# uibk-uncover/ws-unet

Hardware: AMD Instinct MI355X
Metric: 512x512 grayscale images/sec (UNet predict) (higher is better)
Workload: dtype f16 MFMA on the f16 halves + ONE block-scaled fp4 (e2m1) MFMA per tap pair for both residual cross terms (per-pixel / per-(co, tap) E8M0 scales), fp32 accumulate; planar storage

## Files before the change

ws_unet_amd/csrc/planar.hip:

```cpp
#include "wsu_device.h"

namespace {

typedef __attribute__((address_space(3))) void lds_void;
typedef __attribute__((address_space(1))) const void glb_void;

__device__ __forceinline__ void swap32(uint32_t& upper_of, uint32_t& lower_of) {
    const auto r = __builtin_amdgcn_permlane32_swap(upper_of, lower_of, false, false);
    upper_of = r[0]; lower_of = r[1];
}

__device__ __forceinline__ void store_chunk_px(const f32x4& X, const f32x4& Y, char* dst, size_t plane_bytes, int hh, bool ok, float div_lo = WSU_F8_XLO_DIV, bool with_res = true) {
    uint32_t xh0, xh1, xlo, yh0, yh1, ylo;
    wsu_split4_f16r8(X, div_lo, xh0, xh1, xlo);
    wsu_split4_f16r8(Y, div_lo, yh0, yh1, ylo);
    swap32(xh0, yh0); swap32(xh1, yh1);
    uint32_t xlp = xlo, ylp = ylo;
    swap32(xlo, xlp); swap32(ylo, ylp);
    if (ok) {
        *reinterpret_cast<u32x4*>(dst + hh * plane_bytes) = mk_u4(xh0, xh1, yh0, yh1);
        if (with_res && !hh) *reinterpret_cast<u32x4*>(dst + 2 * plane_bytes) = mk_u4(xlo, xlp, ylo, ylp);
    }
}

// ... 386 lines not shown
            const int yy = min(irow, a.h - 1), xx = min(icol, a.w - 1);
#pragma unroll
            for (int cp = 0; cp < 2; ++cp)
#pragma unroll
                for (int pl = 0; pl < 2; ++pl)
                    mk[cp][pl] = *reinterpret_cast<const u32x2*>(a.mask + ((((size_t)cur.n * nci + cur.cb * 4 + mh * 2 + cp) * 3 + pl) * hw + (size_t)yy * a.w + xx) * 16 + hh * 8);
        }
        const char* ldsA = st + GEO::IN1 + (mh * 32 + l31) * 16;
        const char* ldsB = st + (row * 64 + 2 * l31) * 16;
        auto boff = [](int plane, int sub) constexpr { return (((plane * 2 + (sub >> 1)) * 4) * 64 + (sub & 1)) * 16; };
        if constexpr (HONLY) {
#pragma unroll
            for (int s2 = 0; s2 < 4; ++s2) {
                const u32x4 ah = *reinterpret_cast<const u32x4*>(ldsA + ((s2 * 2 + hh) * 64) * 16);
                const u32x4 bh = *reinterpret_cast<const u32x4*>(ldsB + boff(hh, s2));
                wsu_mfma_f16(ah, bh, acc);
            }
        } else {
#pragma unroll
        for (int t = 0; t < 2; ++t) {
            const int s = 2 * t + hh;
            const u32x4 a0 = *reinterpret_cast<const u32x4*>(ldsA + ((s * 4 + 2) * 64) * 16), a1 = *reinterpret_cast<const u32x4*>(ldsA + ((s * 4 + 3) * 64) * 16);
            const u32x4 b0 = *reinterpret_cast<const u32x4*>(ldsB + boff(2, s)), b1 = *reinterpret_cast<const u32x4*>(ldsB + boff(3, s));
            wsu_mfma_f8x2(a0, a1, b0, b1, sc_a, sc_b, acc);
#pragma unroll
            for (int u = 0; u < 2; ++u) {
                const int s2 = 2 * t + u;
                const u32x4 ah = *reinterpret_cast<const u32x4*>(ldsA + ((s2 * 4 + hh) * 64) * 16);
                const u32x4 bh = *reinterpret_cast<const u32x4*>(ldsB + boff(hh, s2));
                wsu_mfma_f16(ah, bh, acc);
            }
        }
        }
        if (c + 1 == a.nch) {
            const bool ok = irow < a.h && icol < a.w;
#pragma unroll
            for (int cp = 0; cp < 2; ++cp) {
                const int oc = cur.cb * 4 + mh * 2 + cp;
                f32x4 X, Y;
#pragma unroll
                for (int e = 0; e < 4; ++e) { X[e] = acc[8 * cp + e]; Y[e] = acc[8 * cp + 4 + e]; }
                if (a.mask) {
#pragma unroll
                    for (int e = 0; e < 4; ++e) {
                        const uint32_t wx = e < 2 ? mk[cp][0].x : mk[cp][0].y, wy = e < 2 ? mk[cp][1].x : mk[cp][1].y;
                        const short hx = (short)((e & 1) ? wx >> 16 : wx & 0xFFFF), hy = (short)((e & 1) ? wy >> 16 : wy & 0xFFFF);
                        if (!(hx > 0)) X[e] = 0.f;
                        if (!(hy > 0)) Y[e] = 0.f;
                    }
                }
                char* dst = a.dx + ((((size_t)cur.n * nci + oc) * 3) * hw + (size_t)min(irow, a.h - 1) * a.w + min(icol, a.w - 1)) * 16;
                store_chunk_px(X, Y, dst, hw * 16, hh, ok, WSU_F8_GLO_DIV, !HONLY);
            }
            ++kt; c = 0;
            if (j + 1 < J) cur = ctb_tile_of(a, lw + kt * G);
        } else {
            ++c;
        }
    }
}

__global__ void pack_convt_dgrad_pl_kernel(const float* __restrict__ w, char* __restrict__ dst, int cin, int cout) {
    const int nch = cout / 16;
    const long long total = (long long)(cin / WSU_COB) * nch * 4 * WSU_COB;
    for (long long d = (long long)blockIdx.x * blockDim.x + threadIdx.x; d < total; d += (long long)gridDim.x * blockDim.x) {
        long long t = d;
        const int m = t % WSU_COB; t /= WSU_COB;
        const int sub = t % 4; t /= 4;
        const int c = t % nch; const int cb = (int)(t / nch);
        f32x4 q[4];
#pragma unroll
        for (int e = 0; e < 16; ++e) q[e >> 2][e & 3] = w[(((size_t)(cb * WSU_COB + m) * cout + c * 16 + e) * 2 + (sub >> 1)) * 2 + (sub & 1)];
        uint32_t h[8], l[4], x[4];
#pragma unroll
        for (int k = 0; k < 4; ++k) wsu_split4_f16f8(q[k], WSU_F8_WLO_DIV, WSU_F8_W_DIV, h[2 * k], h[2 * k + 1], l[k], x[k]);
        char* base = dst + (((size_t)cb * nch + c) * 4 + sub) * (4 * WSU_COB * 16) + m * 16;
        *reinterpret_cast<u32x4*>(base) = mk_u4(h[0], h[1], h[2], h[3]);
        *reinterpret_cast<u32x4*>(base + WSU_COB * 16) = mk_u4(h[4], h[5], h[6], h[7]);
        *reinterpret_cast<u32x4*>(base + 2 * WSU_COB * 16) = mk_u4(x[0], x[1], x[2], x[3]);
        *reinterpret_cast<u32x4*>(base + 3 * WSU_COB * 16) = mk_u4(l[0], l[1], l[2], l[3]);
    }
}

struct FirstPlArgs { const float* x; const float* w; const float* b; char* y; unsigned* range_flag; int n, h, w_, cin, cout, relu; unsigned char* relu_mask_out; int yq; };

template <int FMT, int CINMAX>
__global__ __launch_bounds__(256) void first_pl_kernel(const FirstPlArgs a) {
    constexpr bool YQ = FMT == WSU_PLANAR_Q;
    extern __shared__ __attribute__((aligned(16))) char smem[];
    float* wl = reinterpret_cast<float*>(smem);
    float* bl = wl + a.cin * 9 * a.cout;
    for (int i = threadIdx.x; i < a.cin * 9 * a.cout; i += blockDim.x) {
        const int co = i % a.cout, tap = (i / a.cout) % 9, ci = i / (9 * a.cout);
        wl[i] = a.w[((size_t)co * a.cin + ci) * 9 + tap];
    }
    for (int i = threadIdx.x; i < a.cout; i += blockDim.x) bl[i] = a.b ? a.b[i] : 0.f;
    __syncthreads();
    const size_t hw = (size_t)a.h * a.w_;
    const long long total = (long long)a.n * hw;
    const int nco = a.cout >> 4;
    float vmax = 0.f;
    for (long long i = (long long)blockIdx.x * blockDim.x + threadIdx.x; i < total; i += (long long)gridDim.x * blockDim.x) {
        const int x = (int)(i % a.w_); long long t = i / a.w_;
        const int y = (int)(t % a.h); const int img = (int)(t / a.h);
        float p[CINMAX][9];
#pragma unroll
        for (int ci = 0; ci < CINMAX; ++ci)
            if (ci < a.cin) {
                const float* src = a.x + ((size_t)img * a.cin + ci) * hw;
#pragma unroll
                for (int tp = 0; tp < 9; ++tp)
                    p[ci][tp] = src[(size_t)wsu_reflect(y + tp / 3 - 1, a.h) * a.w_ + wsu_reflect(x + tp % 3 - 1, a.w_)];
            }
        for (int oc = 0; oc < nco; ++oc) {
            f32x2 acc2[8];
#pragma unroll
            for (int k = 0; k < 8; ++k) acc2[k] = *reinterpret_cast<const f32x2*>(bl + oc * 16 + 2 * k);
#pragma unroll
            for (int ci = 0; ci < CINMAX; ++ci)
                if (ci < a.cin)
#pragma unroll
                    for (int tp = 0; tp < 9; ++tp) {
                        const float* wr = wl + (ci * 9 + tp) * a.cout + oc * 16;
                        const f32x2 pw = {p[ci][tp & ~1], p[ci][(tp | 1) < 9 ? (tp | 1) : tp]};
#pragma unroll
                        for (int g = 0; g < 4; ++g) {
                            const f32x4 w4 = *reinterpret_cast<const f32x4*>(wr + 4 * g);
                            const f32x2 wlo = {w4[0], w4[1]}, whi = {w4[2], w4[3]};
                            if (tp & 1) {
                                asm volatile("v_pk_fma_f32 %0, %1, %2, %0 op_sel:[1,0,0] op_sel_hi:[1,1,1]" : "+v"(acc2[2 * g]) : "v"(pw), "v"(wlo));
                                asm volatile("v_pk_fma_f32 %0, %1, %2, %0 op_sel:[1,0,0] op_sel_hi:[1,1,1]" : "+v"(acc2[2 * g + 1]) : "v"(pw), "v"(whi));
                            } else {
                                asm volatile("v_pk_fma_f32 %0, %1, %2, %0 op_sel:[0,0,0] op_sel_hi:[0,1,1]" : "+v"(acc2[2 * g]) : "v"(pw), "v"(wlo));
                                asm volatile("v_pk_fma_f32 %0, %1, %2, %0 op_sel:[0,0,0] op_sel_hi:[0,1,1]" : "+v"(acc2[2 * g + 1]) : "v"(pw), "v"(whi));
                            }
                        }
                    }
            asm volatile("s_nop 0" ::: "memory");
            f32x4 v[4];
#pragma unroll
            for (int g = 0; g < 4; ++g) v[g] = mk_f4(acc2[2 * g][0], acc2[2 * g][1], acc2[2 * g + 1][0], acc2[2 * g + 1][1]);
            uint32_t h[8], lo[4];
#pragma unroll
            for (int g = 0; g < 4; ++g) {
                if (a.relu) {
#pragma unroll
                    for (int e = 0; e < 4; ++e) v[g][e] = fmaxf(v[g][e], 0.f);
                }
#pragma unroll
                for (int e = 0; e < 4; ++e) vmax = fmaxf(vmax, fabsf(v[g][e]));
            }
            if constexpr (YQ) {
                u32x4 h0, h1, qg; uint32_t sb;
                wsu_q4_encode16(v, h0, h1, qg, sb);
                char* chunk = a.y + ((size_t)img * nco + oc) * wsu_q_chunk_bytes(a.h, a.w_);
                char* dq = chunk + ((size_t)y * a.w_ + x) * 16;
                *reinterpret_cast<u32x4*>(dq) = h0;
                *reinterpret_cast<u32x4*>(dq + hw * 16) = h1;
                *reinterpret_cast<u32x4*>(dq + 2 * hw * 16) = qg;
                *reinterpret_cast<unsigned char*>(chunk + 3 * hw * 16 + wsu_q_soff(y, x, (a.w_ + 31) >> 5)) = (unsigned char)sb;
                continue;
            }
            if constexpr (FMT == WSU_PLANAR_H) {
#pragma unroll
                for (int g = 0; g < 4; ++g) {
                    const f32x2 p0 = {v[g][0], v[g][1]}, p1 = {v[g][2], v[g][3]};
                    h[2 * g] = __builtin_bit_cast(uint32_t, __builtin_convertvector(p0, f16x2)); h[2 * g + 1] = __builtin_bit_cast(uint32_t, __builtin_convertvector(p1, f16x2));
                }
                char* dh = a.y + ((size_t)img * nco + oc) * wsu_h_chunk_bytes(a.h, a.w_) + ((size_t)y * a.w_ + x) * 16;
                *reinterpret_cast<u32x4*>(dh) = mk_u4(h[0], h[1], h[2], h[3]);
                *reinterpret_cast<u32x4*>(dh + hw * 16) = mk_u4(h[4], h[5], h[6], h[7]);
                continue;
            }
#pragma unroll
            for (int g = 0; g < 4; ++g) wsu_split4_f16r8(v[g], WSU_F8_XLO_DIV, h[2 * g], h[2 * g + 1], lo[g]);
            char* dst = a.y + ((((size_t)img * nco + oc) * 3) * hw + (size_t)y * a.w_ + x) * 16;
            *reinterpret_cast<u32x4*>(dst) = mk_u4(h[0], h[1], h[2], h[3]);
            *reinterpret_cast<u32x4*>(dst + hw * 16) = mk_u4(h[4], h[5], h[6], h[7]);
            *reinterpret_cast<u32x4*>(dst + 2 * hw * 16) = mk_u4(lo[0], lo[1], lo[2], lo[3]);
            if (a.relu_mask_out) {
                unsigned char* m = a.relu_mask_out + (((size_t)img * (nco * 2) + oc * 2) * wsu_mask_hp(a.h) + y) * wsu_mask_wp(a.w_) + x;
                m[0] = (unsigned char)wsu_f16x8_pos_bits(mk_u4(h[0], h[1], h[2], h[3]));
                m[(size_t)wsu_mask_hp(a.h) * wsu_mask_wp(a.w_)] = (unsigned char)wsu_f16x8_pos_bits(mk_u4(h[4], h[5], h[6], h[7]));
            }
        }
    }
    if (a.range_flag && !(vmax <= (FMT == WSU_PLANAR_H ? WSU_F16_RANGE : WSU_F8_RANGE))) atomicOr(a.range_flag, 1u);
}

}

extern "C" {

int wsu_convt2x2_pl_fwd(const void* x, const void* w_packed, const float* bias, void* y, int n, int h, int w, int cin, int cout,
                        int y_format, unsigned* range_flag, void* stream) {
    WSU_REQUIRE(y_format == WSU_PLANAR_A || y_format == WSU_PLANAR_Q, "convt2x2_pl: y_format must be WSU_PLANAR_A or WSU_PLANAR_Q");
    WSU_REQUIRE(x && w_packed && y, "convt2x2_pl: null pointer");
    WSU_REQUIRE(n > 0 && h > 0 && w > 0, "convt2x2_pl: bad shape n=%d h=%d w=%d", n, h, w);
    WSU_REQUIRE(cin > 0 && cin % 32 == 0, "convt2x2_pl: cin=%d must be a multiple of 32", cin);
    WSU_REQUIRE(cout > 0 && cout % WSU_COB == 0 && cout <= 1024, "convt2x2_pl: cout=%d must be a multiple of %d (<= 1024)", cout, WSU_COB);
    WSU_REQUIRE((long long)h * w * 200 < 0xFFFFFFF0LL, "convt2x2_pl: h*w too large (two input chunks and one output chunk must stay below 4 GiB)");
    CtpArgs a;
    a.x = (const char*)x; a.wp = (const char*)w_packed; a.bias = bias; a.y = (char*)y; a.range_flag = range_flag;
    a.n = n; a.h = h; a.w = w; a.cin = cin; a.cout = cout; a.yq = y_format == WSU_PLANAR_Q ? 1 : 0;
    a.tiles_x = (w + ct::TW - 1) / ct::TW; a.tiles_y = (h + ct::TH - 1) / ct::TH; a.ncb = cout / WSU_COB; a.nst = cin / 32;
    const long long nt = (long long)n * a.tiles_x * a.tiles_y * a.ncb;
    WSU_REQUIRE(nt > 0 && nt < 0x3FFFFFFFLL, "convt2x2_pl: %lld tiles out of range", nt);
    a.ntiles = (int)nt;
    const int ncu = wsu_cu_count("convt2x2_pl");
    if (!ncu) return WSU_ERR_HIP;
    static bool attr_done = false;
    if (!attr_done) {
        if (int rc = wsu_raise_lds(convt2x2_pl_kernel<false>, ct::LDS_TOTAL, "convt2x2_pl")) return rc;
        if (int rc = wsu_raise_lds(convt2x2_pl_kernel<true>, ct::LDS_TOTAL, "convt2x2_pl")) return rc;
        attr_done = true;
    }
    const int grid = (int)(nt < ncu ? nt : ncu);
    if (a.yq) hipLaunchKernelGGL(convt2x2_pl_kernel<true>, dim3(grid), dim3(ct::NT), ct::LDS_TOTAL, static_cast<hipStream_t>(stream), a);
    else hipLaunchKernelGGL(convt2x2_pl_kernel<false>, dim3(grid), dim3(ct::NT), ct::LDS_TOTAL, static_cast<hipStream_t>(stream), a);
    return wsu_check_launch("convt2x2_pl_kernel");
}

int wsu_convt2x2_pl_pack_dgrad(const float* w_iohw, void* w_packed, int cin, int cout, void* stream) {
    WSU_REQUIRE(w_iohw && w_packed, "convt2x2_pl_pack_dgrad: null pointer");
    WSU_REQUIRE(cin > 0 && cin % WSU_COB == 0 && cout > 0 && cout % 16 == 0, "convt2x2_pl_pack_dgrad: bad channels cin=%d cout=%d", cin, cout);
    hipLaunchKernelGGL(pack_convt_dgrad_pl_kernel, dim3(256), dim3(256), 0, static_cast<hipStream_t>(stream), w_iohw, (char*)w_packed, cin, cout);
    return wsu_check_launch("pack_convt_dgrad_pl_kernel");
}

int wsu_convt2x2_pl_bwd_data(const void* dy, const void* w_packed_dgrad, void* dx, const void* mask,
                             int n, int h, int w, int cin, int cout, int products, void* stream) {
    WSU_REQUIRE(dy && w_packed_dgrad && dx, "convt2x2_pl_bwd_data: null pointer");
    WSU_REQUIRE(products == WSU_PRODUCTS_F16F8 || products == WSU_PRODUCTS_F16, "convt2x2_pl_bwd_data: products must be WSU_PRODUCTS_F16F8 or WSU_PRODUCTS_F16");
    WSU_REQUIRE(n > 0 && h > 0 && w > 0 && cin > 0 && cin % WSU_COB == 0 && cout > 0 && cout % 16 == 0, "convt2x2_pl_bwd_data: bad shape (cin %% 64, cout %% 16)");
    WSU_REQUIRE((long long)h * w * 192 < 0xFFFFFFF0LL, "convt2x2_pl_bwd_data: h*w too large (a plane triple of dy must stay below 4 GiB)");
    CtbPlArgs a;
    a.dy = (const char*)dy; a.wp = (const char*)w_packed_dgrad; a.dx = (char*)dx; a.mask = (const char*)mask;
    a.n = n; a.h = h; a.w = w; a.cin = cin; a.cout = cout;
    a.tiles_x = (w + ctb::TW - 1) / ctb::TW; a.tiles_y = (h + ctb::TH - 1) / ctb::TH; a.ncb = cin / WSU_COB; a.nch = cout / 16;
    const long long nt = (long long)n * a.tiles_x * a.tiles_y * a.ncb;
    WSU_REQUIRE(nt > 0 && nt < 0x3FFFFFFFLL, "convt2x2_pl_bwd_data: %lld tiles out of range", nt);
    a.ntiles = (int)nt;
    const int ncu = wsu_cu_count("convt2x2_pl_bwd_data");
    if (!ncu) return WSU_ERR_HIP;
    static bool attr_done = false;
    if (!attr_done) {
        if (int rc = wsu_raise_lds(convt2x2_bwd_pl_kernel<false>, CtbGeo<false>::LDS_TOTAL, "convt2x2_bwd_pl")) return rc;
        if (int rc = wsu_raise_lds(convt2x2_bwd_pl_kernel<true>, CtbGeo<true>::LDS_TOTAL, "convt2x2_bwd_pl")) return rc;
        attr_done = true;
    }
    const int grid = (int)(nt < ncu ? nt : ncu);
    if (products == WSU_PRODUCTS_F16) hipLaunchKernelGGL(convt2x2_bwd_pl_kernel<true>, dim3(grid), dim3(ctb::NT), CtbGeo<true>::LDS_TOTAL, static_cast<hipStream_t>(stream), a);
    else hipLaunchKernelGGL(convt2x2_bwd_pl_kernel<false>, dim3(grid), dim3(ctb::NT), CtbGeo<false>::LDS_TOTAL, static_cast<hipStream_t>(stream), a);
    return wsu_check_launch("convt2x2_bwd_pl_kernel");
}

int wsu_conv3x3_first_pl_fwd(const float* x_nchw, const float* w_oihw, const float* bias, void* y, int n, int h, int w, int cin, int cout,
                             int relu, int y_format, unsigned* range_flag, unsigned char* relu_mask_out, void* stream) {
    WSU_REQUIRE(y_format == WSU_PLANAR_A || y_format == WSU_PLANAR_Q || y_format == WSU_PLANAR_H, "conv3x3_first_pl: y_format must be WSU_PLANAR_A, WSU_PLANAR_Q or WSU_PLANAR_H");
    WSU_REQUIRE(!(relu_mask_out && y_format != WSU_PLANAR_A), "conv3x3_first_pl: relu_mask_out belongs to the training forward (format WSU_PLANAR_A)");
    WSU_REQUIRE((long long)h * w * 50 < 0xFFFFFFF0LL, "conv3x3_first_pl: h*w too large");
    WSU_REQUIRE(x_nchw && w_oihw && y, "conv3x3_first_pl: null pointer");
    WSU_REQUIRE(n > 0 && h >= 2 && w >= 2 && cin >= 1 && cin <= 8 && cout > 0 && cout % 16 == 0 && cout <= 128, "conv3x3_first_pl: bad shape");
    WSU_REQUIRE(!relu_mask_out || (long long)n * (cout / 8) * wsu_mask_hp(h) * wsu_mask_wp(w) < 0x7FFFFFF0LL, "conv3x3_first_pl: mask plane too large");
    FirstPlArgs a{x_nchw, w_oihw, bias, (char*)y, range_flag, n, h, w, cin, cout, relu, relu_mask_out, y_format == WSU_PLANAR_Q ? 1 : 0};
    const long long total = (long long)n * h * w;
    const unsigned nblk = (unsigned)((total + 255) / 256 < 16384 ? (total + 255) / 256 : 16384);
    const size_t lds = ((size_t)cin * 9 * cout + cout) * sizeof(float);
    hipStream_t s_ = static_cast<hipStream_t>(stream);
    if (cin == 1) {
        if (y_format == WSU_PLANAR_H) hipLaunchKernelGGL((first_pl_kernel<WSU_PLANAR_H, 1>), dim3(nblk), dim3(256), lds, s_, a);
        else if (a.yq) hipLaunchKernelGGL((first_pl_kernel<WSU_PLANAR_Q, 1>), dim3(nblk), dim3(256), lds, s_, a);
        else hipLaunchKernelGGL((first_pl_kernel<WSU_PLANAR_A, 1>), dim3(nblk), dim3(256), lds, s_, a);
    } else {
        if (y_format == WSU_PLANAR_H) hipLaunchKernelGGL((first_pl_kernel<WSU_PLANAR_H, 8>), dim3(nblk), dim3(256), lds, s_, a);
        else if (a.yq) hipLaunchKernelGGL((first_pl_kernel<WSU_PLANAR_Q, 8>), dim3(nblk), dim3(256), lds, s_, a);
        else hipLaunchKernelGGL((first_pl_kernel<WSU_PLANAR_A, 8>), dim3(nblk), dim3(256), lds, s_, a);
    }
    return wsu_check_launch("first_pl_kernel");
}

}
```

ws_unet_amd/csrc/wsu_device.h:

```cpp
#pragma once
#include <hip/hip_runtime.h>
#include <stdint.h>
#include <type_traits>
#include "../../include/wsu.h"

typedef __attribute__((ext_vector_type(8))) __bf16 bf16x8;
typedef __attribute__((ext_vector_type(16))) float f32x16;
typedef __attribute__((ext_vector_type(4))) float f32x4;
typedef __attribute__((ext_vector_type(4))) uint32_t u32x4;
typedef __attribute__((ext_vector_type(2))) uint32_t u32x2;
__host__ __device__ __forceinline__ u32x4 mk_u4(uint32_t a, uint32_t b, uint32_t c, uint32_t d) { u32x4 v = {a, b, c, d}; return v; }
__host__ __device__ __forceinline__ u32x2 mk_u2(uint32_t a, uint32_t b) { u32x2 v = {a, b}; return v; }
__host__ __device__ __forceinline__ f32x4 mk_f4(float a, float b, float c, float d) { f32x4 v = {a, b, c, d}; return v; }

void wsu_set_error(const char* fmt, ...);
int wsu_check_launch(const char* what);
#define WSU_REQUIRE(cond, ...)            \
    do {                                  \
        if (!(cond)) {                    \
            wsu_set_error(__VA_ARGS__);   \
            return WSU_ERR_ARG;           \
        }                                 \
    } while (0)
#define WSU_INTERNAL extern "C" __attribute__((visibility("hidden")))
// ... 149 lines not shown
    asm volatile("v_cvt_scalef32_pk_fp4_f16 %0, %1, %2 op_sel:[0,0,1,0]" : "+v"(d) : "v"(h.y), "v"(scale));
    asm volatile("v_cvt_scalef32_pk_fp4_f16 %0, %1, %2 op_sel:[0,0,0,1]" : "+v"(d) : "v"(h.z), "v"(scale));
    asm volatile("v_cvt_scalef32_pk_fp4_f16 %0, %1, %2 op_sel:[0,0,1,1]" : "+v"(d) : "v"(h.w), "v"(scale));
    return d;
}
__host__ __device__ inline size_t wsu_q_sblocks(int h, int w) { return (size_t)((h + 15) >> 4) * (size_t)((w + 31) >> 5); }
__host__ __device__ inline size_t wsu_q_chunk_bytes(int h, int w) { return (size_t)48 * h * w + 512 * wsu_q_sblocks(h, w); }
__device__ __forceinline__ unsigned wsu_q_soff(int y, int x, int tiles_x) {
    return (unsigned)(((y >> 4) * tiles_x + (x >> 5)) * 512 + (y & 15) * 32 + (x & 31));
}
__device__ __forceinline__ void wsu_swap32(uint32_t& upper_of, uint32_t& lower_of) {
    const auto r = __builtin_amdgcn_permlane32_swap(upper_of, lower_of, false, false);
    upper_of = r[0]; lower_of = r[1];
}
__device__ __forceinline__ void wsu_q4_pre_cvt(const f32x4& X, const f32x4& Y, uint32_t& xh0, uint32_t& xh1, uint32_t& yh0, uint32_t& yh1) {
    const f32x2 xa = {X[0], X[1]}, xb = {X[2], X[3]}, ya = {Y[0], Y[1]}, yb = {Y[2], Y[3]};
    xh0 = __builtin_bit_cast(uint32_t, __builtin_convertvector(xa, f16x2)); xh1 = __builtin_bit_cast(uint32_t, __builtin_convertvector(xb, f16x2));
    yh0 = __builtin_bit_cast(uint32_t, __builtin_convertvector(ya, f16x2)); yh1 = __builtin_bit_cast(uint32_t, __builtin_convertvector(yb, f16x2));
}
__device__ __forceinline__ void wsu_q4_pre_enc(const f32x4& X, const f32x4& Y, uint32_t xh0, uint32_t xh1, uint32_t yh0, uint32_t yh1, uint32_t mb,
                                               u32x4& g, uint32_t& dhi, uint32_t& dres, uint32_t& sb) {
    const float r0 = wsu_sub_f16_lo(X[0], xh0), r1 = wsu_sub_f16_hi(X[1], xh0), r2 = wsu_sub_f16_lo(X[2], xh1), r3 = wsu_sub_f16_hi(X[3], xh1);
    const float r4 = wsu_sub_f16_lo(Y[0], yh0), r5 = wsu_sub_f16_hi(Y[1], yh0), r6 = wsu_sub_f16_lo(Y[2], yh1), r7 = wsu_sub_f16_hi(Y[3], yh1);
    uint32_t mw = mb, mp = mb;
    wsu_swap32(mw, mp);
    const int e = wsu_q4_block_exp(mw > mp ? mw : mp);
    const float sc = wsu_pow2f(e), scr = wsu_pow2f(e - 11);
    sb = (uint32_t)(e + 127);
    uint32_t dh = 0, dr = 0;
    asm volatile("v_cvt_scalef32_pk_fp4_f16 %0, %1, %2" : "+v"(dh) : "v"(xh0), "v"(sc));
    asm volatile("v_cvt_scalef32_pk_fp4_f16 %0, %1, %2 op_sel:[0,0,1,0]" : "+v"(dh) : "v"(xh1), "v"(sc));
    asm volatile("v_cvt_scalef32_pk_fp4_f16 %0, %1, %2 op_sel:[0,0,0,1]" : "+v"(dh) : "v"(yh0), "v"(sc));
    asm volatile("v_cvt_scalef32_pk_fp4_f16 %0, %1, %2 op_sel:[0,0,1,1]" : "+v"(dh) : "v"(yh1), "v"(sc));
    dr = __builtin_amdgcn_cvt_scalef32_pk_fp4_f32(dr, r0, r1, scr, 0);
    dr = __builtin_amdgcn_cvt_scalef32_pk_fp4_f32(dr, r2, r3, scr, 1);
    dr = __builtin_amdgcn_cvt_scalef32_pk_fp4_f32(dr, r4, r5, scr, 2);
    dr = __builtin_amdgcn_cvt_scalef32_pk_fp4_f32(dr, r6, r7, scr, 3);
    dhi = dh; dres = dr;
    wsu_swap32(xh0, yh0); wsu_swap32(xh1, yh1);
    g = mk_u4(xh0, xh1, yh0, yh1);
}
__device__ __forceinline__ float wsu_q4_pre(const f32x4& X, const f32x4& Y, u32x4& g, uint32_t& dhi, uint32_t& dres, uint32_t& sb) {
    uint32_t xh0, xh1, yh0, yh1;
    wsu_q4_pre_cvt(X, Y, xh0, xh1, yh0, yh1);
    float mx = __builtin_fmaxf(__builtin_fmaxf(__builtin_fabsf(X[0]), __builtin_fabsf(X[1])), __builtin_fabsf(X[2]));
    mx = __builtin_fmaxf(__builtin_fmaxf(mx, __builtin_fabsf(X[3])), __builtin_fabsf(Y[0]));
    mx = __builtin_fmaxf(__builtin_fmaxf(mx, __builtin_fabsf(Y[1])), __builtin_fabsf(Y[2]));
    mx = __builtin_fmaxf(mx, __builtin_fabsf(Y[3]));
    const f32x2 mm = {mx, 0.f};
    wsu_q4_pre_enc(X, Y, xh0, xh1, yh0, yh1, __builtin_bit_cast(uint32_t, __builtin_convertvector(mm, f16x2)), g, dhi, dres, sb);
    return mx;
}
__device__ __forceinline__ void wsu_q4_pre_bits(const f32x4& X, const f32x4& Y, u32x4& g, uint32_t& dhi, uint32_t& dres, uint32_t& sb) {
    uint32_t xh0, xh1, yh0, yh1;
    wsu_q4_pre_cvt(X, Y, xh0, xh1, yh0, yh1);
    u16x2_t m = __builtin_elementwise_max(__builtin_bit_cast(u16x2_t, xh0 & 0x7FFF7FFFu), __builtin_bit_cast(u16x2_t, xh1 & 0x7FFF7FFFu));
    m = __builtin_elementwise_max(m, __builtin_bit_cast(u16x2_t, yh0 & 0x7FFF7FFFu));
    m = __builtin_elementwise_max(m, __builtin_bit_cast(u16x2_t, yh1 & 0x7FFF7FFFu));
    wsu_q4_pre_enc(X, Y, xh0, xh1, yh0, yh1, m.x > m.y ? m.x : m.y, g, dhi, dres, sb);
}
__device__ __forceinline__ float wsu_max3(float a, float b, float c) {
    float r; asm volatile("v_max3_f32 %0, %1, %2, %3" : "=v"(r) : "v"(a), "v"(b), "v"(c)); return r;
}
__device__ __forceinline__ u32x4 wsu_q4_pair(uint32_t dhi0, uint32_t dres0, uint32_t dhi1, uint32_t dres1) {
    wsu_swap32(dhi0, dhi1); wsu_swap32(dres0, dres1);
    return mk_u4(__builtin_amdgcn_perm(dhi1, dhi0, 0x05040100u), __builtin_amdgcn_perm(dhi1, dhi0, 0x07060302u),
                 __builtin_amdgcn_perm(dres1, dres0, 0x05040100u), __builtin_amdgcn_perm(dres1, dres0, 0x07060302u));
}
__device__ __forceinline__ u32x4 wsu_q4_single(uint32_t dhi, uint32_t dres) {
    uint32_t ph = dhi, pr = dres;
    wsu_swap32(dhi, ph); wsu_swap32(dres, pr);
    return mk_u4(__builtin_amdgcn_perm(ph, dhi, 0x05040100u), __builtin_amdgcn_perm(ph, dhi, 0x07060302u),
                 __builtin_amdgcn_perm(pr, dres, 0x05040100u), __builtin_amdgcn_perm(pr, dres, 0x07060302u));
}
#define WSU_F16_RANGE 65504.f
__host__ __device__ inline size_t wsu_h_chunk_bytes(int h, int w) { return (size_t)32 * h * w; }
__device__ __forceinline__ u32x4 wsu_h_granule(const f32x4& X, const f32x4& Y) {
    const f32x2 xa = {X[0], X[1]}, xb = {X[2], X[3]}, ya = {Y[0], Y[1]}, yb = {Y[2], Y[3]};
    uint32_t xh0 = __builtin_bit_cast(uint32_t, __builtin_convertvector(xa, f16x2)), xh1 = __builtin_bit_cast(uint32_t, __builtin_convertvector(xb, f16x2));
    uint32_t yh0 = __builtin_bit_cast(uint32_t, __builtin_convertvector(ya, f16x2)), yh1 = __builtin_bit_cast(uint32_t, __builtin_convertvector(yb, f16x2));
    wsu_swap32(xh0, yh0); wsu_swap32(xh1, yh1);
    return mk_u4(xh0, xh1, yh0, yh1);
}
__device__ __forceinline__ void wsu_q4_encode16(const f32x4 (&v)[4], u32x4& h0, u32x4& h1, u32x4& q, uint32_t& sb) {
    uint32_t h[8]; float r[16];
#pragma unroll
    for (int k = 0; k < 4; ++k) {
        const f32x2 a = {v[k][0], v[k][1]}, b = {v[k][2], v[k][3]};
        h[2 * k] = __builtin_bit_cast(uint32_t, __builtin_convertvector(a, f16x2)); h[2 * k + 1] = __builtin_bit_cast(uint32_t, __builtin_convertvector(b, f16x2));
        r[4 * k] = wsu_sub_f16_lo(v[k][0], h[2 * k]); r[4 * k + 1] = wsu_sub_f16_hi(v[k][1], h[2 * k]);
        r[4 * k + 2] = wsu_sub_f16_lo(v[k][2], h[2 * k + 1]); r[4 * k + 3] = wsu_sub_f16_hi(v[k][3], h[2 * k + 1]);
    }
    h0 = mk_u4(h[0], h[1], h[2], h[3]); h1 = mk_u4(h[4], h[5], h[6], h[7]);
    const int e = wsu_q4_block_exp(wsu_f16x16_max_abs_bits(h0, h1));
    const float sc = wsu_pow2f(e), scr = wsu_pow2f(e - 11);
    sb = (uint32_t)(e + 127);
    uint32_t q2 = 0, q3 = 0;
    q2 = __builtin_amdgcn_cvt_scalef32_pk_fp4_f32(q2, r[0], r[1], scr, 0); q2 = __builtin_amdgcn_cvt_scalef32_pk_fp4_f32(q2, r[2], r[3], scr, 1);
    q2 = __builtin_amdgcn_cvt_scalef32_pk_fp4_f32(q2, r[4], r[5], scr, 2); q2 = __builtin_amdgcn_cvt_scalef32_pk_fp4_f32(q2, r[6], r[7], scr, 3);
    q3 = __builtin_amdgcn_cvt_scalef32_pk_fp4_f32(q3, r[8], r[9], scr, 0); q3 = __builtin_amdgcn_cvt_scalef32_pk_fp4_f32(q3, r[10], r[11], scr, 1);
    q3 = __builtin_amdgcn_cvt_scalef32_pk_fp4_f32(q3, r[12], r[13], scr, 2); q3 = __builtin_amdgcn_cvt_scalef32_pk_fp4_f32(q3, r[14], r[15], scr, 3);
    q = mk_u4(wsu_f16x8_to_fp4(h0, sc), wsu_f16x8_to_fp4(h1, sc), q2, q3);
}
__device__ __forceinline__ void wsu_mfma_q4(const u32x4& a, const u32x4& b, int scale_a, int scale_b, f32x16& acc) {
    const i32x8 av = {(int)a.x, (int)a.y, (int)a.z, (int)a.w, 0, 0, 0, 0}, bv = {(int)b.x, (int)b.y, (int)b.z, (int)b.w, 0, 0, 0, 0};
    acc = __builtin_amdgcn_mfma_scale_f32_32x32x64_f8f6f4(av, bv, acc, 4, 4, 0, scale_a, 0, scale_b);
}

__device__ __forceinline__ f32x16 wsu_mfma_q4_z(const u32x4& a, const u32x4& b, int scale_a, int scale_b) {
    const i32x8 av = {(int)a.x, (int)a.y, (int)a.z, (int)a.w, 0, 0, 0, 0}, bv = {(int)b.x, (int)b.y, (int)b.z, (int)b.w, 0, 0, 0, 0};
    const f32x16 z = {0.f, 0.f, 0.f, 0.f, 0.f, 0.f, 0.f, 0.f, 0.f, 0.f, 0.f, 0.f, 0.f, 0.f, 0.f, 0.f};
    return __builtin_amdgcn_mfma_scale_f32_32x32x64_f8f6f4(av, bv, z, 4, 4, 0, scale_a, 0, scale_b);
}

__device__ __forceinline__ u32x2 wsu_f16x8_to_fp8_grad(const u32x4& h) {
    const _Float16 m = (_Float16)112.f;
    const f16x8 lim = {m, m, m, m, m, m, m, m};
    const f16x8 c = __builtin_elementwise_max(__builtin_elementwise_min(__builtin_bit_cast(f16x8, h), lim), -lim);
    i16x2 lo = {0, 0}, hi = {0, 0};
    lo = __builtin_amdgcn_cvt_scalef32_pk_fp8_f16(lo, __builtin_shufflevector(c, c, 0, 1), WSU_F8_G_DIV, false);
    lo = __builtin_amdgcn_cvt_scalef32_pk_fp8_f16(lo, __builtin_shufflevector(c, c, 2, 3), WSU_F8_G_DIV, true);
    hi = __builtin_amdgcn_cvt_scalef32_pk_fp8_f16(hi, __builtin_shufflevector(c, c, 4, 5), WSU_F8_G_DIV, false);
    hi = __builtin_amdgcn_cvt_scalef32_pk_fp8_f16(hi, __builtin_shufflevector(c, c, 6, 7), WSU_F8_G_DIV, true);
    return mk_u2(__builtin_bit_cast(uint32_t, lo), __builtin_bit_cast(uint32_t, hi));
}
__device__ __forceinline__ void wsu_mfma_f16(const u32x4& a, const u32x4& b, f32x16& acc) {
    acc = __builtin_amdgcn_mfma_f32_32x32x16_f16(__builtin_bit_cast(f16x8, a), __builtin_bit_cast(f16x8, b), acc, 0, 0, 0);
}
__device__ __forceinline__ f32x16 wsu_mfma_f16_z(const u32x4& a, const u32x4& b) {
    const f32x16 z = {0.f, 0.f, 0.f, 0.f, 0.f, 0.f, 0.f, 0.f, 0.f, 0.f, 0.f, 0.f, 0.f, 0.f, 0.f, 0.f};
    return __builtin_amdgcn_mfma_f32_32x32x16_f16(__builtin_bit_cast(f16x8, a), __builtin_bit_cast(f16x8, b), z, 0, 0, 0);
}
__device__ __forceinline__ void wsu_mfma_f8x2(const u32x4& a_blk0, const u32x4& a_blk1, const u32x4& b_blk0, const u32x4& b_blk1,
                                              int scale_a, int scale_b, f32x16& acc) {
    i32x8 a = {(int)a_blk0.x, (int)a_blk0.y, (int)a_blk0.z, (int)a_blk0.w, (int)a_blk1.x, (int)a_blk1.y, (int)a_blk1.z, (int)a_blk1.w};
    i32x8 b = {(int)b_blk0.x, (int)b_blk0.y, (int)b_blk0.z, (int)b_blk0.w, (int)b_blk1.x, (int)b_blk1.y, (int)b_blk1.z, (int)b_blk1.w};
    acc = __builtin_amdgcn_mfma_scale_f32_32x32x64_f8f6f4(a, b, acc, 0, 0, 0, scale_a, 0, scale_b);
}

__device__ __forceinline__ float wsu_bf16_to_f32(uint16_t v) { return __builtin_bit_cast(float, (uint32_t)v << 16); }

template <int MODE>
__device__ __forceinline__ void wsu_mfma_step(const u32x4& a, const u32x4& b, f32x16& acc) {
    if constexpr (MODE == WSU_MODE_F32) {
        const f32x4 af = __builtin_bit_cast(f32x4, a), bf = __builtin_bit_cast(f32x4, b);
        acc = __builtin_amdgcn_mfma_f32_32x32x2f32(af[0], bf[0], acc, 0, 0, 0);
        acc = __builtin_amdgcn_mfma_f32_32x32x2f32(af[1], bf[1], acc, 0, 0, 0);
        acc = __builtin_amdgcn_mfma_f32_32x32x2f32(af[2], bf[2], acc, 0, 0, 0);
        acc = __builtin_amdgcn_mfma_f32_32x32x2f32(af[3], bf[3], acc, 0, 0, 0);
    } else {
        acc = __builtin_amdgcn_mfma_f32_32x32x16_bf16(__builtin_bit_cast(bf16x8, a), __builtin_bit_cast(bf16x8, b), acc, 0, 0, 0);
    }
}

template <int N> struct wsu_static_for_t {
    template <class F> __device__ __forceinline__ static void run(F&& f) {
        wsu_static_for_t<N - 1>::run(f);
        f(std::integral_constant<int, N - 1>{});
    }
};
template <> struct wsu_static_for_t<0> { template <class F> __device__ __forceinline__ static void run(F&&) {} };
#define WSU_STATIC_FOR(N, VAR, ...) wsu_static_for_t<N>::run([&](auto VAR##_c) __attribute__((always_inline)) { constexpr int VAR = decltype(VAR##_c)::value; __VA_ARGS__ })

__device__ __forceinline__ unsigned wsu_xcd_remap(unsigned bid, unsigned nwg) {
    const unsigned q = nwg >> 3, r = nwg & 7u, xcd = bid & 7u, k = bid >> 3;
    const unsigned base = xcd < r ? xcd * (q + 1) : r * (q + 1) + (xcd - r) * q;
    return base + k;
}
```

Baseline: 3746.

## Restructure first conv kernel with row-blocked sliding windows and buffer stores

Rewrites the first 3x3 conv kernel so each thread computes P=4 consecutive output rows for cin==1, sharing a loaded input window across rows instead of reloading nine taps per pixel. It uses a 3D grid mapping waves to column/row groups, and raw buffer loads and stores with precomputed offsets. The bias is folded into the first FMA, and ReLU is specialized at compile time with max3-based absmax. For the Q format, the block exponent comes from the fp32 max rather than re-scanning the f16 halves, which may round slightly differently. The first layer is likely a small share of the whole UNet time, so the end-to-end gain is limited.

Result: no change. 3777, median of 6 (+0.8%).

```diff
diff --git a/ws_unet_amd/csrc/planar.hip b/ws_unet_amd/csrc/planar.hip
--- a/ws_unet_amd/csrc/planar.hip
+++ b/ws_unet_amd/csrc/planar.hip
@@ -492,106 +492,179 @@
     }
 }
 
-struct FirstPlArgs { const float* x; const float* w; const float* b; char* y; unsigned* range_flag; int n, h, w_, cin, cout, relu; unsigned char* relu_mask_out; int yq; };
-
-template <int FMT, int CINMAX>
+struct FirstPlArgs { const float* x; const float* w; const float* b; char* y; unsigned* range_flag; int n, h, w_, cin, cout, relu; unsigned char* relu_mask_out; int yq;
+                     int wxs; };
+
+constexpr int FIRST_PL_ROWS = 4;
+
+__device__ __forceinline__ float first_max3_abs(float a, float b, float c) {
+    float r; asm("v_max3_f32 %0, |%1|, |%2|, |%3|" : "=v"(r) : "v"(a), "v"(b), "v"(c)); return r;
+}
+
+template <bool HI, bool FIRST>
+__device__ __forceinline__ void first_pk_fma(f32x2& acc, const f32x2& pw, const f32x2& w, const f32x2& c) {
+    if constexpr (FIRST) {
+        if constexpr (HI) asm volatile("v_pk_fma_f32 %0, %1, %2, %3 op_sel:[1,0,0] op_sel_hi:[1,1,1]" : "=v"(acc) : "v"(pw), "v"(w), "v"(c));
+        else asm volatile("v_pk_fma_f32 %0, %1, %2, %3 op_sel:[0,0,0] op_sel_hi:[0,1,1]" : "=v"(acc) : "v"(pw), "v"(w), "v"(c));
+    } else {
+        if constexpr (HI) asm volatile("v_pk_fma_f32 %0, %1, %2, %0 op_sel:[1,0,0] op_sel_hi:[1,1,1]" : "+v"(acc) : "v"(pw), "v"(w));
+        else asm volatile("v_pk_fma_f32 %0, %1, %2, %0 op_sel:[0,0,0] op_sel_hi:[0,1,1]" : "+v"(acc) : "v"(pw), "v"(w));
+    }
+}
+
+template <int P, int TP, bool FIRST>
+__device__ __forceinline__ void first_tap(f32x2 (&acc)[P][8], const f32x2 (&win)[(3 * (P + 2) + 1) / 2], const float* wr, const f32x2 (&bias)[8]) {
+    f32x4 w4[4];
+#pragma unroll
+    for (int g = 0; g < 4; ++g) w4[g] = *reinterpret_cast<const f32x4*>(wr + 4 * g);
+#pragma unroll
+    for (int r = 0; r < P; ++r)
+#pragma unroll
+        for (int g = 0; g < 4; ++g) {
+            const f32x2 wlo = {w4[g][0], w4[g][1]}, whi = {w4[g][2], w4[g][3]};
+            const f32x2& pw = win[(3 * r + TP) >> 1];
+            if ((3 * r + TP) & 1) {
+                first_pk_fma<true, FIRST>(acc[r][2 * g], pw, wlo, bias[2 * g]);
+                first_pk_fma<true, FIRST>(acc[r][2 * g + 1], pw, whi, bias[2 * g + 1]);
+            } else {
+                first_pk_fma<false, FIRST>(acc[r][2 * g], pw, wlo, bias[2 * g]);
+                first_pk_fma<false, FIRST>(acc[r][2 * g + 1], pw, whi, bias[2 * g + 1]);
+            }
+        }
+}
+template <int P, bool FIRST>
+__device__ __forceinline__ void first_plane(f32x2 (&acc)[P][8], const f32x2 (&win)[(3 * (P + 2) + 1) / 2], const float* wr, const f32x2 (&bias)[8]) {
+    first_tap<P, 0, FIRST>(acc, win, wr, bias);
+    first_tap<P, 1, false>(acc, win, wr + 16, bias); first_tap<P, 2, false>(acc, win, wr + 32, bias);
+    first_tap<P, 3, false>(acc, win, wr + 48, bias); first_tap<P, 4, false>(acc, win, wr + 64, bias);
+    first_tap<P, 5, false>(acc, win, wr + 80, bias); first_tap<P, 6, false>(acc, win, wr + 96, bias);
+    first_tap<P, 7, false>(acc, win, wr + 112, bias); first_tap<P, 8, false>(acc, win, wr + 128, bias);
+}
+
+template <int FMT, int CINMAX, int P, bool RELU>
 __global__ __launch_bounds__(256) void first_pl_kernel(const FirstPlArgs a) {
     constexpr bool YQ = FMT == WSU_PLANAR_Q;
+    constexpr int NPAIR = (3 * (P + 2) + 1) / 2;
     extern __shared__ __attribute__((aligned(16))) char smem[];
     float* wl = reinterpret_cast<float*>(smem);
-    float* bl = wl + a.cin * 9 * a.cout;
-    for (int i = threadIdx.x; i < a.cin * 9 * a.cout; i += blockDim.x) {
-        const int co = i % a.cout, tap = (i / a.cout) % 9, ci = i / (9 * a.cout);
-        wl[i] = a.w[((size_t)co * a.cin + ci) * 9 + tap];
-    }
-    for (int i = threadIdx.x; i < a.cout; i += blockDim.x) bl[i] = a.b ? a.b[i] : 0.f;
+    const int rows = 1 + a.cin * 9, nco = a.cout >> 4;
+    for (int oc = 0; oc < nco; ++oc)
+        for (int row = threadIdx.x >> 4; row < rows; row += 16) {
+            const int co = oc * 16 + (threadIdx.x & 15);
+            wl[(oc * rows + row) * 16 + (threadIdx.x & 15)] = row ? a.w[(size_t)co * (rows - 1) + (row - 1)] : a.b ? a.b[co] : 0.f;
+        }
     __syncthreads();
-    const size_t hw = (size_t)a.h * a.w_;
-    const long long total = (long long)a.n * hw;
-    const int nco = a.cout >> 4;
+    const int wave = __builtin_amdgcn_readfirstlane((int)(threadIdx.x >> 6));
+    const int x = (int)((((blockIdx.x << a.wxs) + (wave & ((1 << a.wxs) - 1))) << 6) + (threadIdx.x & 63));
+    if (x >= a.w_) return;
+    const int wys = 2 - a.wxs;
+    const int nrg = (a.h + P - 1) / P;
+    const unsigned hw = (unsigned)a.h * (unsigned)a.w_, hw16 = hw * 16u;
+    const int xo[3] = {wsu_reflect(x - 1, a.w_) * 4, x * 4, wsu_reflect(x + 1, a.w_) * 4};
+    const int xs = (x >> 5) * 512 + (x & 31);
+    const int tiles_x = (a.w_ + 31) >> 5;
+    const int mhp = wsu_mask_hp(a.h), mwp = wsu_mask_wp(a.w_);
+    const unsigned cbytes = FMT == WSU_PLANAR_H ? (unsigned)wsu_h_chunk_bytes(a.h, a.w_) : YQ ? (unsigned)wsu_q_chunk_bytes(a.h, a.w_) : 3u * hw16;
     float vmax = 0.f;
-    for (long long i = (long long)blockIdx.x * blockDim.x + threadIdx.x; i < total; i += (long long)gridDim.x * blockDim.x) {
-        const int x = (int)(i % a.w_); long long t = i / a.w_;
-        const int y = (int)(t % a.h); const int img = (int)(t / a.h);
-        float p[CINMAX][9];
-#pragma unroll
-        for (int ci = 0; ci < CINMAX; ++ci)
-            if (ci < a.cin) {
-                const float* src = a.x + ((size_t)img * a.cin + ci) * hw;
-#pragma unroll
-                for (int tp = 0; tp < 9; ++tp)
-                    p[ci][tp] = src[(size_t)wsu_reflect(y + tp / 3 - 1, a.h) * a.w_ + wsu_reflect(x + tp % 3 - 1, a.w_)];
+    for (int img = blockIdx.z; img < a.n; img += gridDim.z) {
+        const auto rs_m = __builtin_amdgcn_make_buffer_rsrc(a.relu_mask_out ? a.relu_mask_out + (size_t)img * (nco * 2) * mhp * mwp : nullptr, 0,
+                                                            a.relu_mask_out ? nco * 2 * mhp * mwp : 0, 0x00020000);
+        for (int rg = (int)(blockIdx.y << wys) + (wave >> a.wxs); rg < nrg; rg += (int)(gridDim.y << wys)) {
+            const int y0 = rg * P;
+            f32x2 win[CINMAX][NPAIR];
+#pragma unroll
+            for (int ci = 0; ci < CINMAX; ++ci)
+                if (ci < a.cin) {
+                    const auto rs_x = __builtin_amdgcn_make_buffer_rsrc(const_cast<float*>(a.x + ((size_t)img * a.cin + ci) * hw), 0, (int)(hw * 4u), 0x00020000);
+                    if (3 * (P + 2) & 1) win[ci][NPAIR - 1][1] = 0.f;
+#pragma unroll
+                    for (int k = 0; k < P + 2; ++k) {
+                        const int ro = wsu_reflect(y0 - 1 + k, a.h) * a.w_ * 4;
+#pragma unroll
+                        for (int c = 0; c < 3; ++c)
+                            win[ci][(3 * k + c) >> 1][(3 * k + c) & 1] = __builtin_bit_cast(float, __builtin_amdgcn_raw_buffer_load_b32(rs_x, xo[c], ro, 0));
+                    }
+                }
+            int vo[P][4];
+#pragma unroll
+            for (int r = 0; r < P; ++r) {
+                const int y = y0 + r;
+                vo[r][0] = (int)(((unsigned)y * (unsigned)a.w_ + (unsigned)x) * 16u);
+                vo[r][1] = (int)((unsigned)vo[r][0] + hw16); vo[r][2] = (int)((unsigned)vo[r][0] + 2u * hw16);
+                vo[r][3] = (int)(3u * hw16 + (unsigned)(((y >> 4) * tiles_x) * 512 + (y & 15) * 32 + xs));
+#pragma unroll
+                for (int k = 0; k < (YQ ? 4 : FMT == WSU_PLANAR_H ? 2 : 3); ++k) asm volatile("" : "+v"(vo[r][k]));
             }
-        for (int oc = 0; oc < nco; ++oc) {
-            f32x2 acc2[8];
-#pragma unroll
-            for (int k = 0; k < 8; ++k) acc2[k] = *reinterpret_cast<const f32x2*>(bl + oc * 16 + 2 * k);
-#pragma unroll
-            for (int ci = 0; ci < CINMAX; ++ci)
-                if (ci < a.cin)
-#pragma unroll
-                    for (int tp = 0; tp < 9; ++tp) {
-                        const float* wr = wl + (ci * 9 + tp) * a.cout + oc * 16;
-                        const f32x2 pw = {p[ci][tp & ~1], p[ci][(tp | 1) < 9 ? (tp | 1) : tp]};
+            char* yc = a.y + (size_t)img * nco * cbytes;
+            const float* wc = wl;
+            for (int oc = 0; oc < nco; ++oc, yc += cbytes, wc += rows * 16) {
+                f32x2 acc2[P][8], bias[8];
+#pragma unroll
+                for (int g = 0; g < 4; ++g) {
+                    const f32x4 b4 = *reinterpret_cast<const f32x4*>(wc + 4 * g);
+                    bias[2 * g] = f32x2{b4[0], b4[1]}; bias[2 * g + 1] = f32x2{b4[2], b4[3]};
+                }
+                first_plane<P, true>(acc2, win[0], wc + 16, bias);
+#pragma unroll
+                for (int ci = 1; ci < CINMAX; ++ci)
+                    if (ci < a.cin) first_plane<P, false>(acc2, win[ci], wc + 16 + ci * 144, bias);
+                asm volatile("s_nop 0" ::: "memory");
+                const auto rs = __builtin_amdgcn_make_buffer_rsrc(yc, 0, (int)cbytes, 0x00020000);
+#pragma unroll
+                for (int r = 0; r < P; ++r) {
+                    const int y = y0 + r;
+                    if (r > 0 && y >= a.h) break;
+                    f32x4 v[4];
+#pragma unroll
+                    for (int g = 0; g < 4; ++g) v[g] = mk_f4(acc2[r][2 * g][0], acc2[r][2 * g][1], acc2[r][2 * g + 1][0], acc2[r][2 * g + 1][1]);
+                    float mx = 0.f;
+                    if constexpr (RELU) {
+#pragma unroll
+                        for (int g = 0; g < 4; ++g)
+#pragma unroll
+                            for (int e = 0; e < 4; ++e) { float t; asm("v_max_f32_e32 %0, 0, %1" : "=v"(t) : "v"(v[g][e])); v[g][e] = t; }
+                        mx = first_max3_abs(v[0][0], v[0][1], v[0][2]);
+                        mx = first_max3_abs(mx, v[0][3], v[1][0]); mx = first_max3_abs(mx, v[1][1], v[1][2]); mx = first_max3_abs(mx, v[1][3], v[2][0]);
+                        mx = first_max3_abs(mx, v[2][1], v[2][2]); mx = first_max3_abs(mx, v[2][3], v[3][0]); mx = first_max3_abs(mx, v[3][1], v[3][2]);
+                        mx = first_max3_abs(mx, mx, v[3][3]);
+                        vmax = wsu_max3(vmax, vmax, mx);
+                    } else {
+#pragma unroll
+                        for (int g = 0; g < 4; ++g)
+#pragma unroll
+                            for (int e = 0; e < 4; ++e) vmax = fmaxf(vmax, fabsf(v[g][e]));
+                    }
+                    if constexpr (YQ) {
+                        u32x4 h0, h1, qg; uint32_t sb; float res[16];
+                        wsu_q4_split16(v, h0, h1, res);
+                        wsu_q4_finish16(h0, h1, res, RELU ? wsu_f16_bits_of_max(mx) : wsu_f16x16_max_abs_bits(h0, h1), qg, sb);
+                        __builtin_amdgcn_raw_buffer_store_b128(h0, rs, vo[r][0], 0, 0);
+                        __builtin_amdgcn_raw_buffer_store_b128(h1, rs, vo[r][1], 0, 0);
+                        __builtin_amdgcn_raw_buffer_store_b128(qg, rs, vo[r][2], 0, 0);
+                        __builtin_amdgcn_raw_buffer_store_b8((unsigned char)sb, rs, vo[r][3], 0, 0);
+                    } else if constexpr (FMT == WSU_PLANAR_H) {
+                        uint32_t h[8];
 #pragma unroll
                         for (int g = 0; g < 4; ++g) {
-                            const f32x4 w4 = *reinterpret_cast<const f32x4*>(wr + 4 * g);
-                            const f32x2 wlo = {w4[0], w4[1]}, whi = {w4[2], w4[3]};
-                            if (tp & 1) {
-                                asm volatile("v_pk_fma_f32 %0, %1, %2, %0 op_sel:[1,0,0] op_sel_hi:[1,1,1]" : "+v"(acc2[2 * g]) : "v"(pw), "v"(wlo));
-                                asm volatile("v_pk_fma_f32 %0, %1, %2, %0 op_sel:[1,0,0] op_sel_hi:[1,1,1]" : "+v"(acc2[2 * g + 1]) : "v"(pw), "v"(whi));
-                            } else {
-                                asm volatile("v_pk_fma_f32 %0, %1, %2, %0 op_sel:[0,0,0] op_sel_hi:[0,1,1]" : "+v"(acc2[2 * g]) : "v"(pw), "v"(wlo));
-                                asm volatile("v_pk_fma_f32 %0, %1, %2, %0 op_sel:[0,0,0] op_sel_hi:[0,1,1]" : "+v"(acc2[2 * g + 1]) : "v"(pw), "v"(whi));
-                            }
+                            const f32x2 p0 = {v[g][0], v[g][1]}, p1 = {v[g][2], v[g][3]};
+                            h[2 * g] = __builtin_bit_cast(uint32_t, __builtin_convertvector(p0, f16x2)); h[2 * g + 1] = __builtin_bit_cast(uint32_t, __builtin_convertvector(p1, f16x2));
+                        }
+                        __builtin_amdgcn_raw_buffer_store_b128(mk_u4(h[0], h[1], h[2], h[3]), rs, vo[r][0], 0, 0);
+                        __builtin_amdgcn_raw_buffer_store_b128(mk_u4(h[4], h[5], h[6], h[7]), rs, vo[r][1], 0, 0);
+                    } else {
+                        uint32_t h[8], lo[4];
+#pragma unroll
+                        for (int g = 0; g < 4; ++g) wsu_split4_f16r8(v[g], WSU_F8_XLO_DIV, h[2 * g], h[2 * g + 1], lo[g]);
+                        __builtin_amdgcn_raw_buffer_store_b128(mk_u4(h[0], h[1], h[2], h[3]), rs, vo[r][0], 0, 0);
+                        __builtin_amdgcn_raw_buffer_store_b128(mk_u4(h[4], h[5], h[6], h[7]), rs, vo[r][1], 0, 0);
+                        __builtin_amdgcn_raw_buffer_store_b128(mk_u4(lo[0], lo[1], lo[2], lo[3]), rs, vo[r][2], 0, 0);
+                        if (a.relu_mask_out) {
+                            const int mo = (oc * 2 * mhp + y) * mwp;
+                            __builtin_amdgcn_raw_buffer_store_b8((unsigned char)wsu_f16x8_pos_bits(mk_u4(h[0], h[1], h[2], h[3])), rs_m, mo + x, 0, 0);
+                            __builtin_amdgcn_raw_buffer_store_b8((unsigned char)wsu_f16x8_pos_bits(mk_u4(h[4], h[5], h[6], h[7])), rs_m, mo + mhp * mwp + x, 0, 0);
                         }
                     }
-            asm volatile("s_nop 0" ::: "memory");
-            f32x4 v[4];
-#pragma unroll
-            for (int g = 0; g < 4; ++g) v[g] = mk_f4(acc2[2 * g][0], acc2[2 * g][1], acc2[2 * g + 1][0], acc2[2 * g + 1][1]);
-            uint32_t h[8], lo[4];
-#pragma unroll
-            for (int g = 0; g < 4; ++g) {
-                if (a.relu) {
-#pragma unroll
-                    for (int e = 0; e < 4; ++e) v[g][e] = fmaxf(v[g][e], 0.f);
                 }
-#pragma unroll
-                for (int e = 0; e < 4; ++e) vmax = fmaxf(vmax, fabsf(v[g][e]));
-            }
-            if constexpr (YQ) {
-                u32x4 h0, h1, qg; uint32_t sb;
-                wsu_q4_encode16(v, h0, h1, qg, sb);
-                char* chunk = a.y + ((size_t)img * nco + oc) * wsu_q_chunk_bytes(a.h, a.w_);
-                char* dq = chunk + ((size_t)y * a.w_ + x) * 16;
-                *reinterpret_cast<u32x4*>(dq) = h0;
-                *reinterpret_cast<u32x4*>(dq + hw * 16) = h1;
-                *reinterpret_cast<u32x4*>(dq + 2 * hw * 16) = qg;
-                *reinterpret_cast<unsigned char*>(chunk + 3 * hw * 16 + wsu_q_soff(y, x, (a.w_ + 31) >> 5)) = (unsigned char)sb;
-                continue;
-            }
-            if constexpr (FMT == WSU_PLANAR_H) {
-#pragma unroll
-                for (int g = 0; g < 4; ++g) {
-                    const f32x2 p0 = {v[g][0], v[g][1]}, p1 = {v[g][2], v[g][3]};
-                    h[2 * g] = __builtin_bit_cast(uint32_t, __builtin_convertvector(p0, f16x2)); h[2 * g + 1] = __builtin_bit_cast(uint32_t, __builtin_convertvector(p1, f16x2));
-                }
-                char* dh = a.y + ((size_t)img * nco + oc) * wsu_h_chunk_bytes(a.h, a.w_) + ((size_t)y * a.w_ + x) * 16;
-                *reinterpret_cast<u32x4*>(dh) = mk_u4(h[0], h[1], h[2], h[3]);
-                *reinterpret_cast<u32x4*>(dh + hw * 16) = mk_u4(h[4], h[5], h[6], h[7]);
-                continue;
-            }
-#pragma unroll
-            for (int g = 0; g < 4; ++g) wsu_split4_f16r8(v[g], WSU_F8_XLO_DIV, h[2 * g], h[2 * g + 1], lo[g]);
-            char* dst = a.y + ((((size_t)img * nco + oc) * 3) * hw + (size_t)y * a.w_ + x) * 16;
-            *reinterpret_cast<u32x4*>(dst) = mk_u4(h[0], h[1], h[2], h[3]);
-            *reinterpret_cast<u32x4*>(dst + hw * 16) = mk_u4(h[4], h[5], h[6], h[7]);
-            *reinterpret_cast<u32x4*>(dst + 2 * hw * 16) = mk_u4(lo[0], lo[1], lo[2], lo[3]);
-            if (a.relu_mask_out) {
-                unsigned char* m = a.relu_mask_out + (((size_t)img * (nco * 2) + oc * 2) * wsu_mask_hp(a.h) + y) * wsu_mask_wp(a.w_) + x;
-                m[0] = (unsigned char)wsu_f16x8_pos_bits(mk_u4(h[0], h[1], h[2], h[3]));
-                m[(size_t)wsu_mask_hp(a.h) * wsu_mask_wp(a.w_)] = (unsigned char)wsu_f16x8_pos_bits(mk_u4(h[4], h[5], h[6], h[7]));
             }
         }
     }
@@ -673,20 +746,29 @@
     WSU_REQUIRE(x_nchw && w_oihw && y, "conv3x3_first_pl: null pointer");
     WSU_REQUIRE(n > 0 && h >= 2 && w >= 2 && cin >= 1 && cin <= 8 && cout > 0 && cout % 16 == 0 && cout <= 128, "conv3x3_first_pl: bad shape");
     WSU_REQUIRE(!relu_mask_out || (long long)n * (cout / 8) * wsu_mask_hp(h) * wsu_mask_wp(w) < 0x7FFFFFF0LL, "conv3x3_first_pl: mask plane too large");
-    FirstPlArgs a{x_nchw, w_oihw, bias, (char*)y, range_flag, n, h, w, cin, cout, relu, relu_mask_out, y_format == WSU_PLANAR_Q ? 1 : 0};
-    const long long total = (long long)n * h * w;
-    const unsigned nblk = (unsigned)((total + 255) / 256 < 16384 ? (total + 255) / 256 : 16384);
+    FirstPlArgs a{x_nchw, w_oihw, bias, (char*)y, range_flag, n, h, w, cin, cout, relu, relu_mask_out, y_format == WSU_PLANAR_Q ? 1 : 0, 0};
+    constexpr int P1 = FIRST_PL_ROWS, FIRST_PL_MAX_WG = 8192;
+    const int P = cin == 1 ? P1 : 1;
+    a.wxs = w > 128 ? 2 : w > 64 ? 1 : 0;
+    const long long gx = (w + (64 << a.wxs) - 1) / (64 << a.wxs), gz = n < 65535 ? n : 65535;
+    const long long gy_all = ((h + P - 1) / P + (4 >> a.wxs) - 1) / (4 >> a.wxs), gy_cap = FIRST_PL_MAX_WG / (gx * gz) > 1 ? FIRST_PL_MAX_WG / (gx * gz) : 1;
+    const long long gy = gy_all < gy_cap ? gy_all : gy_cap < 65535 ? gy_cap : 65535;
+    const dim3 grid((unsigned)gx, (unsigned)gy, (unsigned)gz);
     const size_t lds = ((size_t)cin * 9 * cout + cout) * sizeof(float);
     hipStream_t s_ = static_cast<hipStream_t>(stream);
-    if (cin == 1) {
-        if (y_format == WSU_PLANAR_H) hipLaunchKernelGGL((first_pl_kernel<WSU_PLANAR_H, 1>), dim3(nblk), dim3(256), lds, s_, a);
-        else if (a.yq) hipLaunchKernelGGL((first_pl_kernel<WSU_PLANAR_Q, 1>), dim3(nblk), dim3(256), lds, s_, a);
-        else hipLaunchKernelGGL((first_pl_kernel<WSU_PLANAR_A, 1>), dim3(nblk), dim3(256), lds, s_, a);
-    } else {
-        if (y_format == WSU_PLANAR_H) hipLaunchKernelGGL((first_pl_kernel<WSU_PLANAR_H, 8>), dim3(nblk), dim3(256), lds, s_, a);
-        else if (a.yq) hipLaunchKernelGGL((first_pl_kernel<WSU_PLANAR_Q, 8>), dim3(nblk), dim3(256), lds, s_, a);
-        else hipLaunchKernelGGL((first_pl_kernel<WSU_PLANAR_A, 8>), dim3(nblk), dim3(256), lds, s_, a);
-    }
+    const auto launch = [&](auto fmt) {
+        constexpr int F = decltype(fmt)::value;
+        if (cin == 1) {
+            if (relu) hipLaunchKernelGGL((first_pl_kernel<F, 1, P1, true>), grid, dim3(256), lds, s_, a);
+            else hipLaunchKernelGGL((first_pl_kernel<F, 1, P1, false>), grid, dim3(256), lds, s_, a);
+        } else {
+            if (relu) hipLaunchKernelGGL((first_pl_kernel<F, 8, 1, true>), grid, dim3(256), lds, s_, a);
+            else hipLaunchKernelGGL((first_pl_kernel<F, 8, 1, false>), grid, dim3(256), lds, s_, a);
+        }
+    };
+    if (y_format == WSU_PLANAR_H) launch(std::integral_constant<int, WSU_PLANAR_H>{});
+    else if (a.yq) launch(std::integral_constant<int, WSU_PLANAR_Q>{});
+    else launch(std::integral_constant<int, WSU_PLANAR_A>{});
     return wsu_check_launch("first_pl_kernel");
 }
 
diff --git a/ws_unet_amd/csrc/wsu_device.h b/ws_unet_amd/csrc/wsu_device.h
--- a/ws_unet_amd/csrc/wsu_device.h
+++ b/ws_unet_amd/csrc/wsu_device.h
@@ -255,8 +255,8 @@
     wsu_swap32(xh0, yh0); wsu_swap32(xh1, yh1);
     return mk_u4(xh0, xh1, yh0, yh1);
 }
-__device__ __forceinline__ void wsu_q4_encode16(const f32x4 (&v)[4], u32x4& h0, u32x4& h1, u32x4& q, uint32_t& sb) {
-    uint32_t h[8]; float r[16];
+__device__ __forceinline__ void wsu_q4_split16(const f32x4 (&v)[4], u32x4& h0, u32x4& h1, float (&r)[16]) {
+    uint32_t h[8];
 #pragma unroll
     for (int k = 0; k < 4; ++k) {
         const f32x2 a = {v[k][0], v[k][1]}, b = {v[k][2], v[k][3]};
@@ -265,7 +265,13 @@
         r[4 * k + 2] = wsu_sub_f16_lo(v[k][2], h[2 * k + 1]); r[4 * k + 3] = wsu_sub_f16_hi(v[k][3], h[2 * k + 1]);
     }
     h0 = mk_u4(h[0], h[1], h[2], h[3]); h1 = mk_u4(h[4], h[5], h[6], h[7]);
-    const int e = wsu_q4_block_exp(wsu_f16x16_max_abs_bits(h0, h1));
+}
+__device__ __forceinline__ uint32_t wsu_f16_bits_of_max(float mx) {
+    const f32x2 mm = {mx, 0.f};
+    return __builtin_bit_cast(uint32_t, __builtin_convertvector(mm, f16x2));
+}
+__device__ __forceinline__ void wsu_q4_finish16(const u32x4& h0, const u32x4& h1, const float (&r)[16], uint32_t mb, u32x4& q, uint32_t& sb) {
+    const int e = wsu_q4_block_exp(mb);
     const float sc = wsu_pow2f(e), scr = wsu_pow2f(e - 11);
     sb = (uint32_t)(e + 127);
     uint32_t q2 = 0, q3 = 0;
@@ -274,6 +280,11 @@
     q3 = __builtin_amdgcn_cvt_scalef32_pk_fp4_f32(q3, r[8], r[9], scr, 0); q3 = __builtin_amdgcn_cvt_scalef32_pk_fp4_f32(q3, r[10], r[11], scr, 1);
     q3 = __builtin_amdgcn_cvt_scalef32_pk_fp4_f32(q3, r[12], r[13], scr, 2); q3 = __builtin_amdgcn_cvt_scalef32_pk_fp4_f32(q3, r[14], r[15], scr, 3);
     q = mk_u4(wsu_f16x8_to_fp4(h0, sc), wsu_f16x8_to_fp4(h1, sc), q2, q3);
+}
+__device__ __forceinline__ void wsu_q4_encode16(const f32x4 (&v)[4], u32x4& h0, u32x4& h1, u32x4& q, uint32_t& sb) {
+    float r[16];
+    wsu_q4_split16(v, h0, h1, r);
+    wsu_q4_finish16(h0, h1, r, wsu_f16x16_max_abs_bits(h0, h1), q, sb);
 }
 __device__ __forceinline__ void wsu_mfma_q4(const u32x4& a, const u32x4& b, int scale_a, int scale_b, f32x16& acc) {
     const i32x8 av = {(int)a.x, (int)a.y, (int)a.z, (int)a.w, 0, 0, 0, 0}, bv = {(int)b.x, (int)b.y, (int)b.z, (int)b.w, 0, 0, 0, 0};
```
